# michaelneale/p2p-llm-tunnel

Measured on AMD Instinct MI355X. Metric: tunneled req/s + added p50 TTFT vs direct, mock-LLM SSE at 1/2/4/8 streams, higher is better.
Workload: dtype n/a

## Files before the change

p2p_llm_tunnel_amd/models/server.py:

```python
from __future__ import annotations

import argparse
import asyncio
import functools
import json
import os
import queue
import socket
import sys
import threading
import time
import uuid
from typing import NamedTuple

import torch


class Sampling:
    __slots__ = ("temperature", "top_k", "top_p", "seed")

    def __init__(self, temperature: float = 0.0, top_k: int = 0, top_p: float = 1.0, seed: int | None = None):
        self.temperature = float(temperature)
        self.top_k = int(top_k)
        self.top_p = float(top_p)
# ... 214 lines not shown
        self.h_lp_ids = torch.zeros((rows, MAX_TOP_LOGPROBS), dtype=torch.int32, pin_memory=cuda)
        self.d_lp = self.d_lp_ids = None
        if device is not None:
            self.d_lp = torch.zeros(self.h_lp.shape, dtype=torch.float32, device=device)
            self.d_lp_ids = torch.zeros(self.h_lp_ids.shape, dtype=torch.int32, device=device)
        self.ev = torch.cuda.Event() if cuda else None
        self.n = 0
        self.emits = []
        self.embeds = []
        self.d_emb = self.h_emb = None


class Engine:

    def __init__(self, device="cuda:0", config="tiny", max_batch=8, seed=0, use_graph=True, rows=64, model=None,
                 small_rows=16, prefix_cache=False, prefix_min=16):
        if model is None:
            from p2p_llm_tunnel_amd.models.tiny_llm import TinyLlama
            model = TinyLlama(config, device=device, max_batch=max_batch, seed=seed, fused=True)
        if prefix_cache and not callable(getattr(model, "kv_copy", None)):
            raise ValueError("prefix_cache needs a model with kv_copy(jobs) (slot-to-slot K/V row copy)")
        use_graph = use_graph and model.device.type == "cuda" and hasattr(model, "step_rows")
        max_batch = getattr(model, "max_batch", max_batch)
        if not (1 <= max_batch <= rows and 1 <= small_rows <= rows):
            raise ValueError("need 1 <= max_batch <= rows and small_rows <= rows")
        self.model = model
        self.device = self.model.device
        self.rows = rows
        self.small_rows = small_rows
        self.use_graph = use_graph
        cuda = self.device.type == "cuda"
        self._k = 0
        self._d_last = torch.zeros(max_batch + 1, dtype=torch.int64, device=self.device)
        sizes = [small_rows] + ([rows] if rows > small_rows else []) if use_graph else [rows]
        lp_dev = self.device if use_graph else None
        self._bufs = {R: [_StepBuf(R, cuda, lp_dev), _StepBuf(R, cuda, lp_dev)] for R in sizes}
        self._d_in = {R: torch.zeros((_IN_ROWS, R), dtype=torch.int64, device=self.device) for R in sizes}
        self._graphs = {(R, par, post): self._capture(self._bufs[R][par], 0 if R == small_rows else max_batch, post)
                        for R in sizes if use_graph for par in (0, 1) for post in (0, 1, 2)}
        self.max_batch = max_batch
        self.pending: queue.Queue = queue.Queue()
        self.slots: list[dict | None] = [None] * max_batch
        self.deliver = None
        self._wake = threading.Event()
        self._stop = threading.Event()
# ... 144 lines not shown
            s = self.slots[i]
            s["gen"] += 1
            fin = s["gen"] >= s["req"].max_new or s["pos"] >= max_seq - 1
            emits.append((r, s["req"], fin, s["gen"] - 1))
            if fin:
                done.append(i)
        for pool in pools:
            s = self.slots[pool[0]]
            if s["pos"] >= len(s["ids"]):
                pool[4] = s["req"]
                done.append(pool[0])
        for i in done:
            self.slots[i] = None
        return rows, emits

    def _step_body(self, b: _StepBuf, n: int, run, sample_rows: int = 0, logprobs: bool = False):
        din = self._d_in[b.rows]
        din.copy_(b.h_in, non_blocking=True)
        d = din[:, :n]
        tok = torch.where(d[_DEC] != 0, self._d_last[d[_SLOT]], d[_TOK])
        ids, logits = run(tok, d[_POS].to(torch.int32), d[_SLOT].to(torch.int32))
        if sample_rows:
            from p2p_llm_tunnel_amd import ops
            ops.sample_(logits[:sample_rows], ids[:sample_rows], din[_SMP])
            if logprobs:
                ops.logprobs_(logits[:sample_rows], ids[:sample_rows], din[_LP], b.d_lp[:sample_rows],
                              b.d_lp_ids[:sample_rows])
                b.h_lp.copy_(b.d_lp, non_blocking=True)
                b.h_lp_ids.copy_(b.d_lp_ids, non_blocking=True)
        self._d_last.index_copy_(0, d[_REC], ids)
        b.h_out[:n].copy_(ids, non_blocking=True)

    def _capture(self, b: _StepBuf, emit_rows: int, post: int):
        from p2p_llm_tunnel_amd.models.tiny_llm import capture
        b.np[:] = 0
        b.np[_SLOT, :] = b.np[_REC, :] = self.model.scratch_slot
        run = functools.partial(self.model.step_rows, emit_rows=emit_rows)
        sample_rows = (emit_rows or b.rows) if post else 0
        graph, _ = capture(lambda: self._step_body(b, b.rows, run, sample_rows, post == 2), self.device)
        torch.cuda.synchronize(self.device)
        return graph

    def _launch(self, rows, emits) -> _StepBuf:
        n, scratch = len(rows), self.model.scratch_slot
        R = self.small_rows if self.use_graph and n <= self.small_rows else self.rows
        par = self._k % 2
        self._k += 1
        b = self._bufs[R][par]
        h = b.np
        h[_TOK, :n] = [r.token for r in rows]
        h[_POS, :n] = [r.pos for r in rows]
        h[_SLOT, :n] = [r.slot for r in rows]
        h[_DEC, :n] = [r.decode for r in rows]
        h[_REC, :n] = [r.slot if r.emit else scratch for r in rows]
# ... 672 lines not shown
```

p2p_llm_tunnel_amd/models/tiny_llm.py:

```python
from __future__ import annotations

import math
from dataclasses import dataclass

import torch
import torch.nn.functional as F

from p2p_llm_tunnel_amd import ops


@dataclass(frozen=True)
class LlamaConfig:
    vocab: int = 32000
    dim: int = 1024
    n_layers: int = 4
    n_heads: int = 16
    n_kv_heads: int = 4
    head_dim: int = 64
    ffn: int = 2816
    max_seq: int = 2048
    eps: float = 1e-5
    rope_theta: float = 10000.0
    qk_norm: bool = False
    qkv_bias: bool = False
# ... 131 lines not shown
            if c.qk_norm:
                ws += [L["q_norm"].contiguous(), L["k_norm"].contiguous()]
            if c.qkv_bias:
                ws += [L["bqkv"][head_perm].contiguous()]
        return ws

    def fused_decoder(self) -> ops.FusedLlamaDecoder:
        if self._fused is None:
            c = self.cfg
            dims = ops.LlamaDims(vocab=c.vocab, dim=c.dim, n_layers=c.n_layers, H=c.n_heads, Hkv=c.n_kv_heads,
                                 D=c.head_dim, ffn=c.ffn, max_seq=c.max_seq, max_batch=self.max_batch + 1, eps=c.eps,
                                 theta=c.rope_theta, qk_norm=int(c.qk_norm), qkv_bias=int(c.qkv_bias))
            self._fused = ops.FusedLlamaDecoder(dims, self.fused_weights(), self.k_cache, self.v_cache)
        return self._fused

    def step_rows(self, tokens, pos, slots=None, emit_rows=0, pos_range=None):
        B = tokens.shape[0]
        if self.fused and B <= ops.MAX_ROWS:
            tokens, pos = tokens.contiguous(), pos.contiguous()
            slots = slots.contiguous() if slots is not None else None
            logits = torch.empty(B, self.cfg.vocab, dtype=torch.bfloat16, device=self.device)
            ids = torch.empty(B, dtype=torch.int64, device=self.device)
            self.fused_decoder().step(tokens, pos, logits, ids, slots, emit_rows)
            return ids, logits
        return self._decode_unfused(tokens, pos, pos_range or (0, self.cfg.max_seq - 1))

    def _decode_unfused(self, tokens, pos, pos_range):
        c = self.cfg
        B = tokens.shape[0]
        lens = pos + 1
        x = self.embed.index_select(0, tokens)
# ... 120 lines not shown
```

p2p_llm_tunnel_amd/ops/__init__.py:

```python
from __future__ import annotations

import ctypes
import math
import os

import torch

HERE = os.path.dirname(os.path.abspath(__file__))
_LIB = None


class LlamaDims(ctypes.Structure):
    _fields_ = [(n, ctypes.c_int) for n in ("vocab", "dim", "n_layers", "H", "Hkv", "D", "ffn", "max_seq",
                                           "max_batch")] + [("eps", ctypes.c_float), ("theta", ctypes.c_float),
                                                            ("qk_norm", ctypes.c_int), ("qkv_bias", ctypes.c_int)]


_INT = ctypes.c_int


class GemmPlan(ctypes.Structure):
    _fields_ = [(n, _INT) for n in ("epi", "nw", "tn", "um", "kpl", "grid_x", "grid_y", "ss_in", "M", "N", "K")]


class AttnPlan(ctypes.Structure):
    _fields_ = [(n, _INT) for n in ("D", "G", "slots", "stride", "grid_y")]


class StepPlan(ctypes.Structure):
    _fields_ = ([("rows", _INT), ("emit_rows", _INT)] +
                [(n, GemmPlan) for n in ("qkv_first", "qkv", "o", "gate_up", "down", "lm_head")] +
                [("attn", AttnPlan), ("am_parts", _INT), ("qk_norm_grid", _INT)])


def lib() -> ctypes.CDLL:
    global _LIB
    if _LIB is None:
        path = os.path.join(HERE, os.environ.get("P2PT_HIP_OPS_LIB", "_hip_ops.so"))
        if not os.path.exists(path):
            from . import build as _b
            _b.build()
        _LIB = ctypes.CDLL(path)
        vp, i, f = ctypes.c_void_p, ctypes.c_int, ctypes.c_float
        _LIB.p2pt_rmsnorm.argtypes = [vp, vp, vp, vp, vp, i, i, f, vp]
        _LIB.p2pt_silu_mul.argtypes = [vp, vp, i, i, vp]
        _LIB.p2pt_rope_qkv_cache.argtypes = [vp, vp, vp, vp, vp, i, i, i, i, i, f, vp]
        _LIB.p2pt_qk_norm_rope_cache.argtypes = [vp, vp, vp, vp, vp, vp, vp, vp, i, i, i, i, i, i, f, f, vp]
        _LIB.p2pt_decode_attention.argtypes = [vp, vp, vp, vp, vp, vp, i, i, i, i, i, i, i, f, vp]
        _LIB.p2pt_argmax.argtypes = [vp, vp, i, i, vp]
        _LIB.p2pt_skinny_gemm.argtypes = [vp, vp, vp, i, i, i, vp]
        _LIB.p2pt_sample.argtypes = [vp, vp, vp, i, i, i, vp]
        _LIB.p2pt_logprobs.argtypes = [vp, vp, vp, vp, vp, i, i, vp]
        _LIB.p2pt_kv_copy.argtypes = [vp, vp, i, i, i, i, i, ctypes.POINTER(ctypes.c_int), vp]
        _LIB.p2pt_max_kv_copy_jobs.argtypes = []
        _LIB.p2pt_embed_pool.argtypes = [vp, i, i, vp, vp, i, vp, i, f, i, ctypes.POINTER(ctypes.c_int), vp]
        _LIB.p2pt_max_embed_jobs.argtypes = []
        _LIB.p2pt_llama_ws_bytes.argtypes = [ctypes.POINTER(LlamaDims)]
        _LIB.p2pt_llama_ws_bytes.restype = ctypes.c_size_t
        szp = ctypes.POINTER(ctypes.c_size_t)
        _LIB.p2pt_llama_ws_layout.argtypes = [ctypes.POINTER(LlamaDims), szp, szp, i]
        _LIB.p2pt_llama_ws_layout.restype = ctypes.c_int
        _LIB.p2pt_llama_decode.argtypes = [ctypes.POINTER(LlamaDims), ctypes.POINTER(vp), vp, vp, vp, vp, vp, i, i,
                                           vp, ctypes.c_size_t, vp, vp, vp]
        _LIB.p2pt_llama_plan.argtypes = [ctypes.POINTER(LlamaDims), i, i, ctypes.POINTER(StepPlan)]
        _LIB.p2pt_attn_span.argtypes = [i, i]
        _LIB.p2pt_max_rows.argtypes = []
        _LIB.p2pt_skinny_bench.argtypes = [vp, vp, vp, i, i, i, i, i, i, vp]
        _LIB.p2pt_attn_bench.argtypes = [vp, vp, vp, vp, i, i, i, i, i, vp, vp, vp, vp, i, vp]
        for fn in ("p2pt_rmsnorm", "p2pt_silu_mul", "p2pt_rope_qkv_cache", "p2pt_decode_attention", "p2pt_argmax",
                   "p2pt_skinny_gemm", "p2pt_llama_decode", "p2pt_sample", "p2pt_logprobs", "p2pt_llama_plan", "p2pt_attn_span",
                   "p2pt_max_rows", "p2pt_skinny_bench", "p2pt_attn_bench", "p2pt_kv_copy", "p2pt_max_kv_copy_jobs",
                   "p2pt_embed_pool", "p2pt_max_embed_jobs", "p2pt_qk_norm_rope_cache"):
            getattr(_LIB, fn).restype = ctypes.c_int
        if _LIB.p2pt_max_rows() != MAX_ROWS:
            raise RuntimeError(f"MAX_ROWS = {MAX_ROWS}, but {path} was built for {_LIB.p2pt_max_rows()} rows")
        if _LIB.p2pt_max_kv_copy_jobs() != MAX_KV_COPY_JOBS:
            raise RuntimeError(f"MAX_KV_COPY_JOBS = {MAX_KV_COPY_JOBS}, but {path} was built for "
                               f"{_LIB.p2pt_max_kv_copy_jobs()} jobs")
        if _LIB.p2pt_max_embed_jobs() != MAX_EMBED_JOBS:
            raise RuntimeError(f"MAX_EMBED_JOBS = {MAX_EMBED_JOBS}, but {path} was built for "
                               f"{_LIB.p2pt_max_embed_jobs()} jobs")
    return _LIB


MAX_ROWS = 64
MAX_KV_COPY_JOBS = 8
MAX_EMBED_JOBS = 16
MAX_TOP_LOGPROBS = 20


def step_plan(dims: LlamaDims, B: int, emit_rows: int = 0) -> StepPlan:
    plan = StepPlan()
    if lib().p2pt_llama_plan(ctypes.byref(dims), B, emit_rows, ctypes.byref(plan)) != 0:
        raise ValueError("dims or row count not supported by the fused decode kernels")
    return plan


def attn_span(length: int, slots: int) -> int:
    return lib().p2pt_attn_span(length, slots)


def loaded_path() -> str:
    return lib()._name


def _stream(t: torch.Tensor):
    return ctypes.c_void_p(torch.cuda.current_stream(t.device).cuda_stream)

# ... 164 lines not shown
    _ok(lib().p2pt_decode_attention(_p(q), _p(k_cache), _p(v_cache), _p(lens), _p(out), _p(ws), B, H, Hkv, D, Smax,
                                    nsplit, chunk, scale, _stream(q)), "decode_attention")
    return out


def argmax(logits: torch.Tensor) -> torch.Tensor:
    _check(logits, torch.bfloat16, "logits")
    if logits.dim() != 2:
        raise ValueError("logits must be [B, V]")
    B, V = logits.shape
    out = torch.empty(B, dtype=torch.int64, device=logits.device)
    _ok(lib().p2pt_argmax(_p(logits), _p(out), B, V, _stream(logits)), "argmax")
    return out


def sample_(logits: torch.Tensor, ids: torch.Tensor, params: torch.Tensor) -> torch.Tensor:
    _check(logits, torch.bfloat16, "logits")
    _check(ids, torch.int64, "ids", logits.device)
    _check(params, torch.int64, "params", logits.device)
    if logits.dim() != 2 or ids.shape != (logits.shape[0],) or params.dim() != 2 or params.shape[0] != 5:
        raise ValueError("need logits [B, V], ids [B], params [5, >= B]")
    B, V = logits.shape
    if params.shape[1] < B:
        raise ValueError("params need a column per row")
    _ok(lib().p2pt_sample(_p(logits), _p(ids), _p(params), B, params.shape[1], V, _stream(logits)), "sample")
    return ids


def logprobs_(logits: torch.Tensor, ids: torch.Tensor, want: torch.Tensor, out_lp: torch.Tensor,
              out_ids: torch.Tensor) -> None:
    _check(logits, torch.bfloat16, "logits")
    _check(ids, torch.int64, "ids", logits.device)
    _check(want, torch.int64, "want", logits.device)
    _check(out_lp, torch.float32, "out_lp", logits.device)
    _check(out_ids, torch.int32, "out_ids", logits.device)
    if logits.dim() != 2 or ids.shape != (logits.shape[0],) or want.dim() != 1:
        raise ValueError("need logits [B, V], ids [B], want [>= B]")
    B, V = logits.shape
    if B < 1 or V < 32:
        raise ValueError("need B >= 1 and V >= 32")
# ... 146 lines not shown
                        raise ValueError(f"layer {L}: q_norm and k_norm must be ({dims.D},)")
        elif dims.qkv_bias:
            n_qkv = (dims.H + 2 * dims.Hkv) * dims.D
            for L in range(dims.n_layers):
                if weights[3 + 7 * L + 6].shape != (n_qkv,):
                    raise ValueError(f"layer {L}: bqkv must be ({n_qkv},)")
        nbytes = lib().p2pt_llama_ws_bytes(ctypes.byref(dims))
        if nbytes == 0:
            raise ValueError("model dims not supported by the fused decode kernels")
        self.weights = weights
        self._wptr = (ctypes.c_void_p * len(weights))(*[t.data_ptr() for t in weights])
        self.ws = torch.zeros(nbytes, dtype=torch.uint8, device=dev)
        self.k_cache, self.v_cache = k_cache, v_cache
        self.device = dev
        self._resid = None

    _WS_BUFFERS = (("resid", torch.bfloat16), ("q", torch.bfloat16), ("attn", torch.bfloat16), ("h", torch.bfloat16),
                   ("ss", torch.float32), ("part_o", torch.float32), ("part_ml", torch.float32),
                   ("am_val", torch.float32), ("am_idx", torch.int32), ("counters", torch.int32),
                   ("qkv", torch.bfloat16))

    def workspace_views(self) -> dict:
        d = self.dims
        n = len(self._WS_BUFFERS)
        off, cnt = (ctypes.c_size_t * n)(), (ctypes.c_size_t * n)()
        if lib().p2pt_llama_ws_layout(ctypes.byref(d), off, cnt, n) != n:
            raise RuntimeError("workspace layout: buffer list out of step with decode_fused.hip")
        views = {}
        for (name, dtype), o, c in zip(self._WS_BUFFERS, off, cnt):
            size = torch.empty(0, dtype=dtype).element_size()
# ... 21 lines not shown
        B = tokens.shape[0]
        if slots is not None:
            _check(slots, torch.int32, "slots", self.device)
            if slots.shape != (B,):
                raise ValueError("slots must be [B]")
        limit = MAX_ROWS if slots is not None else min(MAX_ROWS, d.max_batch)
        if not 0 <= emit_rows <= B:
            raise ValueError("emit_rows must be in 0..B")
        if not 1 <= B <= limit or pos.shape != (B,) or ids.shape != (B,):
            raise ValueError(f"rows must be 1..{limit} with matching pos/ids")
        if logits.shape != (B, d.vocab):
            raise ValueError("logits must be [B, vocab]")
        _ok(lib().p2pt_llama_decode(ctypes.byref(d), self._wptr, _p(self.k_cache), _p(self.v_cache), _p(tokens),
                                    _p(pos), _p(slots), B, emit_rows, _p(self.ws), self.ws.numel(), _p(logits),
                                    _p(ids), _stream(tokens)), "llama_decode")
```

p2p_llm_tunnel_amd/ops/decode_fused.hip:

```cpp
#include "decode_fused_kernels.h"

namespace {

struct LlamaDims {
  int vocab, dim, n_layers, H, Hkv, D, ffn, max_seq, max_batch;
  float eps, theta;
  int qk_norm;
  int qkv_bias;
};

constexpr int kTnResid = 1, kTnStore = 2;
constexpr int kCUs = 256;
constexpr int kMaxKpl = 2;

struct GemmPlan {
  int epi, nw, tn, um, kpl;
  int grid_x, grid_y;
  int ss_in;
  int M, N, K;
};
struct AttnPlan {
  int D, G;
  int slots;
  int stride;
  int grid_y;
};
struct StepPlan {
  int rows, emit_rows;
  GemmPlan qkv_first, qkv, o, gate_up, down, lm_head;
  AttnPlan attn;
  int am_parts;
  int qk_norm_grid;
};

GemmPlan plan_gemm(int epi, int tn, int M, int N, int K, bool k_parts = false, int fixed_nw = 0) {
  GemmPlan p{};
  p.epi = epi, p.tn = tn, p.M = M, p.N = N, p.K = K;
  if (k_parts && tn == 1 && (N >> 4) < kCUs) {
    const int kpl = std::min((N >> 3) >= kCUs ? 1 : 2, kMaxKpl);
    if ((M << kpl) <= 16 && K % (32 << kpl) == 0) p.kpl = kpl;
  }
  const int steps = (K >> p.kpl) >> 5;
  if (steps <= 0) return p;
  p.nw = fixed_nw ? fixed_nw : steps <= 16 ? 4 : 8;
  const int per_wave = (steps + p.nw - 1) / p.nw;
  p.um = per_wave <= 1 ? 1 : per_wave <= 2 ? 2 : 4;
  p.grid_x = N / (tn << tile_cwl(p.kpl));
  p.grid_y = (M + 15) >> 4;
  return p;
}

GemmPlan plan_lm_head(const LlamaDims& d, int rows) {
  return plan_gemm(EPI_ARGMAX, kTnStore, rows, d.vocab, d.dim, false, 4);
}

AttnPlan plan_attn(int B, int H, int Hkv, int D, int max_seq) {
  return {D, Hkv > 0 ? H / Hkv : 0, attn_slots(B, Hkv, max_seq), attn_part_stride(max_seq), B * Hkv};
}

StepPlan plan_step(const LlamaDims& d, int B, int emit_rows) {
  StepPlan p{};
  p.rows = B;
  p.emit_rows = emit_rows <= 0 || emit_rows > B ? B : emit_rows;
  p.qkv = plan_gemm(d.qk_norm ? EPI_STORE : d.qkv_bias ? EPI_ROPE_BIAS : EPI_ROPE, 1, B, (d.H + 2 * d.Hkv) * d.D,
                    d.dim);
  if (d.qk_norm) {
    const int per_wg = qknorm_heads_per_wg(d.D);
    p.qk_norm_grid = (d.H + 2 * d.Hkv + per_wg - 1) / per_wg;
  }
  p.attn = plan_attn(B, d.H, d.Hkv, d.D, d.max_seq);
  p.o = plan_gemm(EPI_RESID, kTnResid, B, d.dim, d.H * d.D, true);
  p.gate_up = plan_gemm(EPI_SILU, 1, B, 2 * d.ffn, d.dim);
  p.down = plan_gemm(EPI_RESID, kTnResid, B, d.dim, d.ffn, true);
  p.lm_head = plan_lm_head(d, p.emit_rows);
  p.qkv_first = p.qkv;
  p.qkv_first.ss_in = 1;
  p.gate_up.ss_in = p.o.grid_x;
// ... 183 lines not shown
  const size_t gemm_bytes[] = {size_t(d.vocab) * dim * 2, size_t(d.H + 2 * d.Hkv) * d.D * dim * 2,
                               2 * ffn * dim * 2, dim * hd * 2, dim * ffn * 2};
  for (size_t b : gemm_bytes)
    if (b >= kOob) return false;
  if (d.Hkv <= 0 || d.H % d.Hkv) return false;
  const int gqa = d.H / d.Hkv;
  if (gqa != 1 && gqa != 2 && (gqa < 4 || gqa > 8)) return false;
  if (d.dim % 32 || (d.H * d.D) % 32 || d.ffn % 32) return false;
  if (d.dim % (16 * kTnResid) || d.vocab % (16 * kTnStore) || d.ffn % 16) return false;
  if (d.max_batch <= 0 || d.max_seq <= 0 || d.n_layers <= 0) return false;
  return true;
}

bool rows_ok(int B) { return B > 0 && B <= kMaxM; }

}

extern "C" {

size_t p2pt_llama_ws_bytes(const LlamaDims* d) {
  if (!dims_ok(*d)) return 0;
  return carve(*d, nullptr).bytes;
}

int p2pt_llama_ws_layout(const LlamaDims* d, size_t* off, size_t* count, int n) {
  if (!dims_ok(*d) || n < WS_NBUF) return 0;
  const WsLayout l = ws_layout(*d);
  for (int b = 0; b < WS_NBUF; b++) {
    off[b] = l.off[b];
    count[b] = l.count[b];
  }
  return WS_NBUF;
}

int p2pt_llama_plan(const LlamaDims* d, int B, int emit_rows, StepPlan* out) {
  if (!dims_ok(*d) || !rows_ok(B)) return int(hipErrorInvalidValue);
  *out = plan_step(*d, B, emit_rows);
  return 0;
}

int p2pt_attn_span(int len, int slots) { return len > 0 && slots > 0 ? attn_span(len, unsigned(slots)) : 0; }

int p2pt_max_rows() { return kMaxM; }

int p2pt_llama_decode(const LlamaDims* dp, const void* const* w, void* k_cache, void* v_cache, const int64_t* tokens,
                      const int* pos, const int* slots, int B, int emit_rows, void* ws, size_t ws_bytes, void* logits,
                      int64_t* ids, void* stream) {
  const LlamaDims d = *dp;
  if (!dims_ok(d) || !rows_ok(B) || (!slots && B > d.max_batch)) return int(hipErrorInvalidValue);
  const Workspace W = carve(d, static_cast<uint8_t*>(ws));
  if (ws_bytes < W.bytes) return int(hipErrorInvalidValue);
  const StepPlan P = plan_step(d, B, emit_rows);
  auto s = static_cast<hipStream_t>(stream);
  const size_t layer_cache = size_t(d.max_batch) * d.max_seq * d.Hkv * d.D;
  hipError_t e;
  auto failed = [&](hipError_t r) { return (e = r) != hipSuccess; };

  hipLaunchKernelGGL(k_embed, dim3(B), dim3(256), 0, s, static_cast<const uint16_t*>(w[0]), tokens, W.resid, W.ss,
                     d.dim, d.vocab);
  if (failed(hipGetLastError())) return int(e);
  for (int L = 0; L < d.n_layers; L++) {
    const void* const* wl = w + 3 + (d.qk_norm ? 8 : d.qkv_bias ? 7 : 6) * L;
    uint16_t* kc = static_cast<uint16_t*>(k_cache) + L * layer_cache;
    uint16_t* vc = static_cast<uint16_t*>(v_cache) + L * layer_cache;
    const GemmPlan& qkv = L ? P.qkv : P.qkv_first;
    const GemmArgs to_qkv = d.qk_norm
                                ? gemm(W.resid, wl[1]) + norm(W.ss, qkv.ss_in, d.eps) + store(W.qkv)
                            : d.qkv_bias
                                ? gemm(W.resid, wl[1]) + norm(W.ss, qkv.ss_in, d.eps) +
                                      rope_bias(d, pos, slots, W.q, kc, vc, wl[6])
                                : gemm(W.resid, wl[1]) + norm(W.ss, qkv.ss_in, d.eps) + rope(d, pos, slots, W.q, kc, vc);
    const GemmArgs to_o = gemm(W.attn, wl[2]) + resid(W.resid, W.ss);
    const GemmArgs to_gate_up = gemm(W.resid, wl[4]) + norm(W.ss, P.gate_up.ss_in, d.eps) + store(W.h);
    const GemmArgs to_down = gemm(W.h, wl[5]) + resid(W.resid, W.ss);
    if (failed(launch(qkv, to_qkv, s))) return int(e);
    if (P.qk_norm_grid) {
      const QkNormArgs qn{W.qkv, static_cast<const uint16_t*>(wl[6]), static_cast<const uint16_t*>(wl[7]), pos, slots,
                          d.max_batch, W.q, kc, vc, d.H, d.Hkv, d.max_seq, d.eps, log2f(d.theta)};
      if (failed(launch_qknorm(P.qk_norm_grid, B, d.D, qn, s))) return int(e);
    }
    if (failed(launch_attn(P.attn, W.q, kc, vc, pos, slots, d.max_batch, W.part_o, W.part_ml, W.counters, W.attn, d.H,
                           d.Hkv, d.max_seq, s)))
      return int(e);
    if (failed(launch(P.o, to_o, s))) return int(e);
    if (failed(launch(P.gate_up, to_gate_up, s))) return int(e);
    if (failed(launch(P.down, to_down, s))) return int(e);
  }
  const GemmArgs to_logits =
      gemm(W.resid, w[2]) + norm(W.ss, P.lm_head.ss_in, d.eps) + argmax(logits, W.am_val, W.am_idx);
  if (failed(launch(P.lm_head, to_logits, s))) return int(e);
  hipLaunchKernelGGL(k_argmax_merge, dim3(P.emit_rows), dim3(256), 0, s, W.am_val, W.am_idx, P.am_parts, ids);
  return int(hipGetLastError());
}

int p2pt_skinny_gemm(const void* x, const void* w, void* out, int M, int N, int K, void* stream) {
  if (!rows_ok(M) || N % 32 || K <= 0 || K % 32) return int(hipErrorInvalidValue);
  const GemmPlan p = plan_gemm(EPI_STORE, 2, M, N, K);
  return int(launch(p, gemm(x, w) + store(out), static_cast<hipStream_t>(stream)));
}

int p2pt_qk_norm_rope_cache(const void* qkv, const int* pos, const int* slots, const void* q_weight,
                            const void* k_weight, void* q, void* k_cache, void* v_cache, int B, int H, int Hkv, int D,
                            int Smax, int nslots, float eps, float theta, void* stream) {
  if (!rows_ok(B) || (D != 64 && D != 128) || H <= 0 || Hkv <= 0 || Smax <= 0 || nslots <= 0)
    return int(hipErrorInvalidValue);
  if ((!slots && B > nslots) || !(theta > 0.f)) return int(hipErrorInvalidValue);
  const QkNormArgs a{static_cast<const uint16_t*>(qkv), static_cast<const uint16_t*>(q_weight),
// ... 33 lines not shown
```

p2p_llm_tunnel_amd/ops/decode_fused_kernels.h:

```cpp
#pragma once
#include "bf16_common.h"

#include <algorithm>

namespace {

using namespace p2pt_gpu;

constexpr int kMaxM = 64;

typedef short frag8 __attribute__((ext_vector_type(8)));
typedef float frag4 __attribute__((ext_vector_type(4)));

enum Epi : int { EPI_STORE = 0, EPI_ROPE = 1, EPI_SILU = 2, EPI_RESID = 3, EPI_ARGMAX = 4, EPI_ROPE_BIAS = 5 };

struct GemmArgs {
  const uint16_t* x;
  const uint16_t* w;
  int M, N, K;
  const float* ss_part;
  int ss_parts;
  float eps;
  uint16_t* out;
  float* ss_out;
// ... 286 lines not shown
        if (m >= a.M || !col_ok) continue;
        const float nv = bf_round(rprev[t][r] + bf_round(v[t][r]));
        a.out[size_t(m) * a.N + n] = uint16_t(f2bf_bits(nv));
        sq[r] += nv * nv;
      }
    }
#pragma unroll
    for (int r = 0; r < 4; r++) {
      sq[r] = row16_sum(sq[r]);
      if (c == 0) a.ss_out[bx * kMaxM + mrow0 + r] = sq[r];
    }
  }
}

__global__ __launch_bounds__(256) void k_argmax_merge(const float* __restrict__ am_val, const int* __restrict__ am_idx,
                                                      int parts, int64_t* __restrict__ ids) {
  const int m = blockIdx.x;
  float b = -INFINITY;
  int i = 0x7fffffff;
  for (int p0 = threadIdx.x; p0 < parts; p0 += 8 * 256) {
    float pv[8];
    int pi[8];
#pragma unroll
    for (int j = 0; j < 8; j++) {
      const int p = p0 + j * 256;
      pv[j] = p < parts ? am_val[p * kMaxM + m] : -INFINITY;
      pi[j] = p < parts ? am_idx[p * kMaxM + m] : 0x7fffffff;
    }
#pragma unroll
    for (int j = 0; j < 8; j++)
      if (pv[j] > b || (pv[j] == b && pi[j] < i)) {
// ... 3 lines not shown
  }
  wave_argmax(b, i);
  __shared__ float sb[4];
  __shared__ int si[4];
  if ((threadIdx.x & 63) == 0) {
    sb[threadIdx.x >> 6] = b;
    si[threadIdx.x >> 6] = i;
  }
  __syncthreads();
  if (threadIdx.x == 0) {
    for (int w = 1; w < 4; w++)
      if (sb[w] > b || (sb[w] == b && si[w] < i)) {
        b = sb[w];
        i = si[w];
      }
    ids[m] = i == 0x7fffffff ? 0 : i;
  }
}

__global__ __launch_bounds__(256) void k_embed(const uint16_t* __restrict__ embed, const int64_t* __restrict__ tok,
                                               uint16_t* __restrict__ resid, float* __restrict__ ss_out, int dim,
                                               int vocab) {
  const int b = blockIdx.x;
  int64_t t = tok[b];
  t = t < 0 ? 0 : (t >= vocab ? vocab - 1 : t);
  const uint4* src = reinterpret_cast<const uint4*>(embed + size_t(t) * dim);
  uint4* dst = reinterpret_cast<uint4*>(resid + size_t(b) * dim);
  float ss = 0.f;
  for (int i = threadIdx.x; i < dim / 8; i += 256) {
    const uint4 v = src[i];
    dst[i] = v;
    float f[8];
    unpack8(v, f);
#pragma unroll
    for (int j = 0; j < 8; j++) ss += f[j] * f[j];
  }
  __shared__ float red[4];
  ss = wave_sum(ss);
  if ((threadIdx.x & 63) == 0) red[threadIdx.x >> 6] = ss;
  __syncthreads();
  if (threadIdx.x == 0) ss_out[b] = red[0] + red[1] + red[2] + red[3];
}

struct QkNormArgs {
  const uint16_t* qkv;
  const uint16_t* gq;
  const uint16_t* gk;
  const int* pos;
  const int* slot;
  int nslots;
  uint16_t* q_out;
  uint16_t* kc;
  uint16_t* vc;
  int H, Hkv, Smax;
  float eps, log2_theta;
};
// ... 278 lines not shown
```

p2p_llm_tunnel_amd/ops/sample.hip:

```cpp
#include "bf16_common.h"

namespace {

using namespace p2pt_gpu;

constexpr int kThreads = 1024, kWaves = kThreads / 64;

__device__ __forceinline__ uint32_t okey(float f) {
  uint32_t u = __float_as_uint(f);
  return (u & 0x80000000u) ? ~u : (u | 0x80000000u);
}

__device__ __forceinline__ uint64_t mix64(uint64_t z) {
  z = (z ^ (z >> 30)) * 0xBF58476D1CE4E5B9ull;
  z = (z ^ (z >> 27)) * 0x94D049BB133111EBull;
  return z ^ (z >> 31);
}

__device__ __forceinline__ float gumbel(uint64_t seed, uint64_t ctr, uint32_t i) {
  uint64_t h = mix64(seed + mix64(ctr * 0x9E3779B97F4A7C15ull + i + 1));
  double u = (double(h >> 11) + 0.5) * (1.0 / 9007199254740992.0);
  return float(-log(-log(u)));
}

// ... 45 lines not shown
#pragma unroll
    for (int q = 0; q < 4; q++) {
      if (run + v[q] >= need || q == 3) {
        dg = 255 - 4 * lane - q;
        ab = run;
        break;
      }
      run += v[q];
    }
    *digit_out = dg;
    *above_out = ab;
  }
}

__global__ __launch_bounds__(kThreads) void k_sample(const uint16_t* __restrict__ logits, int64_t* __restrict__ ids,
                                                     const int64_t* __restrict__ params, int ld, int V) {
  const int row = blockIdx.x;
  const int B = ld;
  const float T = __uint_as_float(uint32_t(params[row]));
  if (!(T >= 1e-4f)) return;
  int64_t k = params[B + row];
  float p = __uint_as_float(uint32_t(params[2 * B + row]));
  const uint64_t seed = uint64_t(params[3 * B + row]), ctr = uint64_t(params[4 * B + row]);
  if (k <= 0 || k > V) k = V;
  if (!(p > 0.f && p < 1.f)) p = 1.f;
  const float invT = 1.0f / T;
  const uint16_t* lr = logits + size_t(row) * V;

  __shared__ float red[kWaves];
  __shared__ uint32_t hist_u[256];
  __shared__ float hist_f[256];
  __shared__ int s_digit;
  __shared__ uint32_t s_above_u;
  __shared__ float s_above_f;
  __shared__ float s_best[kWaves];
// ... 57 lines not shown
  int bi = 0x7fffffff;
  for (int i = threadIdx.x; i < V; i += kThreads) {
    const float zi = bf2f(lr[i]) * invT;
    if (okey(zi) < cut) continue;
    am_take(best, bi, zi + gumbel(seed, ctr, uint32_t(i)), i);
  }
  wave_argmax(best, bi);
  if ((threadIdx.x & 63) == 0) {
    s_best[threadIdx.x >> 6] = best;
    s_bi[threadIdx.x >> 6] = bi;
  }
  __syncthreads();
  if (threadIdx.x == 0) {
    for (int w = 1; w < kWaves; w++) am_take(best, bi, s_best[w], s_bi[w]);
    if (bi != 0x7fffffff) ids[row] = bi;
  }
}

}

extern "C" {

int p2pt_sample(const void* logits, int64_t* ids, const int64_t* params, int B, int ld, int V, void* stream) {
  if (B <= 0 || V <= 0 || ld < B) return int(hipErrorInvalidValue);
  hipLaunchKernelGGL(k_sample, dim3(B), dim3(kThreads), 0, static_cast<hipStream_t>(stream),
                     static_cast<const uint16_t*>(logits), ids, params, ld, V);
  return int(hipGetLastError());
}

}
```

Baseline: 15.97.

## Fold token gather, int32 casts and last-token record into fused decode kernels

Adds a staged decode path in which the embed kernel reads the raw int64 staging block directly. It picks the decode token from the last-token buffer and writes int32 pos/slot rows itself. The argmax-merge or sample kernel then scatters the chosen id back into the last-token buffer. This removes the separate torch.where/gather, dtype cast and index_copy kernels from each captured graph step, so fewer launches run per step. It is on by default when graphs are used, and it adds a new code path with duplicated record logic in the argmax and sample kernels.

Measured after the change: 15.97. No clear change (-0.0%).

```diff
diff --git a/p2p_llm_tunnel_amd/models/server.py b/p2p_llm_tunnel_amd/models/server.py
--- a/p2p_llm_tunnel_amd/models/server.py
+++ b/p2p_llm_tunnel_amd/models/server.py
@@ -252,7 +252,7 @@
 class Engine:
 
     def __init__(self, device="cuda:0", config="tiny", max_batch=8, seed=0, use_graph=True, rows=64, model=None,
-                 small_rows=16, prefix_cache=False, prefix_min=16):
+                 small_rows=16, prefix_cache=False, prefix_min=16, native_step=True):
         if model is None:
             from p2p_llm_tunnel_amd.models.tiny_llm import TinyLlama
             model = TinyLlama(config, device=device, max_batch=max_batch, seed=seed, fused=True)
@@ -267,6 +267,7 @@
         self.rows = rows
         self.small_rows = small_rows
         self.use_graph = use_graph
+        self.native_step = bool(native_step) and use_graph
         cuda = self.device.type == "cuda"
         self._k = 0
         self._d_last = torch.zeros(max_batch + 1, dtype=torch.int64, device=self.device)
@@ -441,21 +442,29 @@
             self.slots[i] = None
         return rows, emits
 
-    def _step_body(self, b: _StepBuf, n: int, run, sample_rows: int = 0, logprobs: bool = False):
+    def _step_body(self, b: _StepBuf, n: int, run, sample_rows: int = 0, logprobs: bool = False,
+                   native: bool = False):
         din = self._d_in[b.rows]
         din.copy_(b.h_in, non_blocking=True)
         d = din[:, :n]
-        tok = torch.where(d[_DEC] != 0, self._d_last[d[_SLOT]], d[_TOK])
-        ids, logits = run(tok, d[_POS].to(torch.int32), d[_SLOT].to(torch.int32))
+        if native:
+            ids, logits = run(None, None, staged=(din, self._d_last, not sample_rows))
+        else:
+            tok = torch.where(d[_DEC] != 0, self._d_last[d[_SLOT]], d[_TOK])
+            ids, logits = run(tok, d[_POS].to(torch.int32), d[_SLOT].to(torch.int32))
         if sample_rows:
             from p2p_llm_tunnel_amd import ops
-            ops.sample_(logits[:sample_rows], ids[:sample_rows], din[_SMP])
+            if native:
+                ops.sample_(logits[:sample_rows], ids[:sample_rows], din[_SMP], din[_REC], self._d_last)
+            else:
+                ops.sample_(logits[:sample_rows], ids[:sample_rows], din[_SMP])
             if logprobs:
                 ops.logprobs_(logits[:sample_rows], ids[:sample_rows], din[_LP], b.d_lp[:sample_rows],
                               b.d_lp_ids[:sample_rows])
                 b.h_lp.copy_(b.d_lp, non_blocking=True)
                 b.h_lp_ids.copy_(b.d_lp_ids, non_blocking=True)
-        self._d_last.index_copy_(0, d[_REC], ids)
+        if not native:
+            self._d_last.index_copy_(0, d[_REC], ids)
         b.h_out[:n].copy_(ids, non_blocking=True)
 
     def _capture(self, b: _StepBuf, emit_rows: int, post: int):
@@ -464,7 +473,8 @@
         b.np[_SLOT, :] = b.np[_REC, :] = self.model.scratch_slot
         run = functools.partial(self.model.step_rows, emit_rows=emit_rows)
         sample_rows = (emit_rows or b.rows) if post else 0
-        graph, _ = capture(lambda: self._step_body(b, b.rows, run, sample_rows, post == 2), self.device)
+        graph, _ = capture(lambda: self._step_body(b, b.rows, run, sample_rows, post == 2, self.native_step),
+                           self.device)
         torch.cuda.synchronize(self.device)
         return graph
 
diff --git a/p2p_llm_tunnel_amd/models/tiny_llm.py b/p2p_llm_tunnel_amd/models/tiny_llm.py
--- a/p2p_llm_tunnel_amd/models/tiny_llm.py
+++ b/p2p_llm_tunnel_amd/models/tiny_llm.py
@@ -169,7 +169,16 @@
             self._fused = ops.FusedLlamaDecoder(dims, self.fused_weights(), self.k_cache, self.v_cache)
         return self._fused
 
-    def step_rows(self, tokens, pos, slots=None, emit_rows=0, pos_range=None):
+    def step_rows(self, tokens, pos, slots=None, emit_rows=0, pos_range=None, staged=None):
+        if staged is not None:
+            block, last, record = staged
+            B = block.shape[1]
+            if not (self.fused and B <= ops.MAX_ROWS):
+                raise ValueError(f"a staged step needs the fused path and at most {ops.MAX_ROWS} rows")
+            logits = torch.empty(B, self.cfg.vocab, dtype=torch.bfloat16, device=self.device)
+            ids = torch.empty(B, dtype=torch.int64, device=self.device)
+            self.fused_decoder().step_staged(block, last, logits, ids, emit_rows, record)
+            return ids, logits
         B = tokens.shape[0]
         if self.fused and B <= ops.MAX_ROWS:
             tokens, pos = tokens.contiguous(), pos.contiguous()
diff --git a/p2p_llm_tunnel_amd/ops/__init__.py b/p2p_llm_tunnel_amd/ops/__init__.py
--- a/p2p_llm_tunnel_amd/ops/__init__.py
+++ b/p2p_llm_tunnel_amd/ops/__init__.py
@@ -30,7 +30,7 @@
 class StepPlan(ctypes.Structure):
     _fields_ = ([("rows", _INT), ("emit_rows", _INT)] +
                 [(n, GemmPlan) for n in ("qkv_first", "qkv", "o", "gate_up", "down", "lm_head")] +
-                [("attn", AttnPlan), ("am_parts", _INT), ("qk_norm_grid", _INT)])
+                [("attn", AttnPlan), ("am_parts", _INT), ("qk_norm_grid", _INT), ("staged", _INT)])
 
 
 def lib() -> ctypes.CDLL:
@@ -50,6 +50,7 @@
         _LIB.p2pt_argmax.argtypes = [vp, vp, i, i, vp]
         _LIB.p2pt_skinny_gemm.argtypes = [vp, vp, vp, i, i, i, vp]
         _LIB.p2pt_sample.argtypes = [vp, vp, vp, i, i, i, vp]
+        _LIB.p2pt_sample_record.argtypes = [vp, vp, vp, vp, vp, i, i, i, vp]
         _LIB.p2pt_logprobs.argtypes = [vp, vp, vp, vp, vp, i, i, vp]
         _LIB.p2pt_kv_copy.argtypes = [vp, vp, i, i, i, i, i, ctypes.POINTER(ctypes.c_int), vp]
         _LIB.p2pt_max_kv_copy_jobs.argtypes = []
@@ -62,7 +63,10 @@
         _LIB.p2pt_llama_ws_layout.restype = ctypes.c_int
         _LIB.p2pt_llama_decode.argtypes = [ctypes.POINTER(LlamaDims), ctypes.POINTER(vp), vp, vp, vp, vp, vp, i, i,
                                            vp, ctypes.c_size_t, vp, vp, vp]
+        _LIB.p2pt_llama_decode_staged.argtypes = [ctypes.POINTER(LlamaDims), ctypes.POINTER(vp), vp, vp, vp, i, vp, vp,
+                                                  i, i, i, vp, ctypes.c_size_t, vp, vp, vp]
         _LIB.p2pt_llama_plan.argtypes = [ctypes.POINTER(LlamaDims), i, i, ctypes.POINTER(StepPlan)]
+        _LIB.p2pt_llama_plan_staged.argtypes = [ctypes.POINTER(LlamaDims), i, i, ctypes.POINTER(StepPlan)]
         _LIB.p2pt_attn_span.argtypes = [i, i]
         _LIB.p2pt_max_rows.argtypes = []
         _LIB.p2pt_skinny_bench.argtypes = [vp, vp, vp, i, i, i, i, i, i, vp]
@@ -70,7 +74,8 @@
         for fn in ("p2pt_rmsnorm", "p2pt_silu_mul", "p2pt_rope_qkv_cache", "p2pt_decode_attention", "p2pt_argmax",
                    "p2pt_skinny_gemm", "p2pt_llama_decode", "p2pt_sample", "p2pt_logprobs", "p2pt_llama_plan", "p2pt_attn_span",
                    "p2pt_max_rows", "p2pt_skinny_bench", "p2pt_attn_bench", "p2pt_kv_copy", "p2pt_max_kv_copy_jobs",
-                   "p2pt_embed_pool", "p2pt_max_embed_jobs", "p2pt_qk_norm_rope_cache"):
+                   "p2pt_embed_pool", "p2pt_max_embed_jobs", "p2pt_qk_norm_rope_cache", "p2pt_llama_decode_staged",
+                   "p2pt_llama_plan_staged", "p2pt_sample_record"):
             getattr(_LIB, fn).restype = ctypes.c_int
         if _LIB.p2pt_max_rows() != MAX_ROWS:
             raise RuntimeError(f"MAX_ROWS = {MAX_ROWS}, but {path} was built for {_LIB.p2pt_max_rows()} rows")
@@ -89,9 +94,10 @@
 MAX_TOP_LOGPROBS = 20
 
 
-def step_plan(dims: LlamaDims, B: int, emit_rows: int = 0) -> StepPlan:
+def step_plan(dims: LlamaDims, B: int, emit_rows: int = 0, staged: bool = False) -> StepPlan:
     plan = StepPlan()
-    if lib().p2pt_llama_plan(ctypes.byref(dims), B, emit_rows, ctypes.byref(plan)) != 0:
+    fn = lib().p2pt_llama_plan_staged if staged else lib().p2pt_llama_plan
+    if fn(ctypes.byref(dims), B, emit_rows, ctypes.byref(plan)) != 0:
         raise ValueError("dims or row count not supported by the fused decode kernels")
     return plan
 
@@ -286,7 +292,8 @@
     return out
 
 
-def sample_(logits: torch.Tensor, ids: torch.Tensor, params: torch.Tensor) -> torch.Tensor:
+def sample_(logits: torch.Tensor, ids: torch.Tensor, params: torch.Tensor, rec: torch.Tensor | None = None,
+            last: torch.Tensor | None = None) -> torch.Tensor:
     _check(logits, torch.bfloat16, "logits")
     _check(ids, torch.int64, "ids", logits.device)
     _check(params, torch.int64, "params", logits.device)
@@ -295,7 +302,15 @@
     B, V = logits.shape
     if params.shape[1] < B:
         raise ValueError("params need a column per row")
-    _ok(lib().p2pt_sample(_p(logits), _p(ids), _p(params), B, params.shape[1], V, _stream(logits)), "sample")
+    if (rec is None) != (last is None):
+        raise ValueError("rec and last go together")
+    if rec is not None:
+        _check(rec, torch.int64, "rec", logits.device)
+        _check(last, torch.int64, "last", logits.device)
+        if rec.dim() != 1 or rec.shape[0] < B or last.dim() != 1 or last.shape[0] < 1:
+            raise ValueError("need rec [>= B] and last [slots >= 1]")
+    _ok(lib().p2pt_sample_record(_p(logits), _p(ids), _p(params), _p(rec), _p(last), B, params.shape[1], V,
+                                 _stream(logits)), "sample")
     return ids
 
 
@@ -472,6 +487,7 @@
         self.k_cache, self.v_cache = k_cache, v_cache
         self.device = dev
         self._resid = None
+        self.rows32 = torch.zeros((3, MAX_ROWS), dtype=torch.int32, device=dev)
 
     _WS_BUFFERS = (("resid", torch.bfloat16), ("q", torch.bfloat16), ("attn", torch.bfloat16), ("h", torch.bfloat16),
                    ("ss", torch.float32), ("part_o", torch.float32), ("part_ml", torch.float32),
@@ -523,3 +539,24 @@
         _ok(lib().p2pt_llama_decode(ctypes.byref(d), self._wptr, _p(self.k_cache), _p(self.v_cache), _p(tokens),
                                     _p(pos), _p(slots), B, emit_rows, _p(self.ws), self.ws.numel(), _p(logits),
                                     _p(ids), _stream(tokens)), "llama_decode")
+
+    def step_staged(self, staged: torch.Tensor, last: torch.Tensor, logits: torch.Tensor, ids: torch.Tensor,
+                    emit_rows: int = 0, record: bool = True) -> None:
+        d = self.dims
+        _check(staged, torch.int64, "staged", self.device)
+        _check(last, torch.int64, "last", self.device)
+        _check(logits, torch.bfloat16, "logits", self.device)
+        _check(ids, torch.int64, "ids", self.device)
+        if staged.dim() != 2 or staged.shape[0] < 5 or not 1 <= staged.shape[1] <= MAX_ROWS:
+            raise ValueError(f"staged must be [>= 5, 1..{MAX_ROWS}]")
+        B = staged.shape[1]
+        if last.shape != (d.max_batch,):
+            raise ValueError(f"last must be [{d.max_batch}] (one entry per cache slot)")
+        if not 0 <= emit_rows <= B:
+            raise ValueError("emit_rows must be in 0..B")
+        if ids.shape != (B,) or logits.shape != (B, d.vocab):
+            raise ValueError("need ids [B] and logits [B, vocab]")
+        _ok(lib().p2pt_llama_decode_staged(ctypes.byref(d), self._wptr, _p(self.k_cache), _p(self.v_cache),
+                                           _p(staged), B, _p(last), _p(self.rows32), int(bool(record)), B, emit_rows, _p(self.ws),
+                                           self.ws.numel(), _p(logits), _p(ids), _stream(staged)),
+            "llama_decode_staged")
diff --git a/p2p_llm_tunnel_amd/ops/decode_fused.hip b/p2p_llm_tunnel_amd/ops/decode_fused.hip
--- a/p2p_llm_tunnel_amd/ops/decode_fused.hip
+++ b/p2p_llm_tunnel_amd/ops/decode_fused.hip
@@ -31,6 +31,7 @@
   AttnPlan attn;
   int am_parts;
   int qk_norm_grid;
+  int staged;
 };
 
 GemmPlan plan_gemm(int epi, int tn, int M, int N, int K, bool k_parts = false, int fixed_nw = 0) {
@@ -58,9 +59,10 @@
   return {D, Hkv > 0 ? H / Hkv : 0, attn_slots(B, Hkv, max_seq), attn_part_stride(max_seq), B * Hkv};
 }
 
-StepPlan plan_step(const LlamaDims& d, int B, int emit_rows) {
+StepPlan plan_step(const LlamaDims& d, int B, int emit_rows, bool staged = false) {
   StepPlan p{};
   p.rows = B;
+  p.staged = staged;
   p.emit_rows = emit_rows <= 0 || emit_rows > B ? B : emit_rows;
   p.qkv = plan_gemm(d.qk_norm ? EPI_STORE : d.qkv_bias ? EPI_ROPE_BIAS : EPI_ROPE, 1, B, (d.H + 2 * d.Hkv) * d.D,
                     d.dim);
@@ -274,51 +276,33 @@
 
 bool rows_ok(int B) { return B > 0 && B <= kMaxM; }
 
-}
-
-extern "C" {
-
-size_t p2pt_llama_ws_bytes(const LlamaDims* d) {
-  if (!dims_ok(*d)) return 0;
-  return carve(*d, nullptr).bytes;
-}
-
-int p2pt_llama_ws_layout(const LlamaDims* d, size_t* off, size_t* count, int n) {
-  if (!dims_ok(*d) || n < WS_NBUF) return 0;
-  const WsLayout l = ws_layout(*d);
-  for (int b = 0; b < WS_NBUF; b++) {
-    off[b] = l.off[b];
-    count[b] = l.count[b];
-  }
-  return WS_NBUF;
-}
-
-int p2pt_llama_plan(const LlamaDims* d, int B, int emit_rows, StepPlan* out) {
-  if (!dims_ok(*d) || !rows_ok(B)) return int(hipErrorInvalidValue);
-  *out = plan_step(*d, B, emit_rows);
-  return 0;
-}
-
-int p2pt_attn_span(int len, int slots) { return len > 0 && slots > 0 ? attn_span(len, unsigned(slots)) : 0; }
-
-int p2pt_max_rows() { return kMaxM; }
-
-int p2pt_llama_decode(const LlamaDims* dp, const void* const* w, void* k_cache, void* v_cache, const int64_t* tokens,
-                      const int* pos, const int* slots, int B, int emit_rows, void* ws, size_t ws_bytes, void* logits,
-                      int64_t* ids, void* stream) {
-  const LlamaDims d = *dp;
-  if (!dims_ok(d) || !rows_ok(B) || (!slots && B > d.max_batch)) return int(hipErrorInvalidValue);
-  const Workspace W = carve(d, static_cast<uint8_t*>(ws));
-  if (ws_bytes < W.bytes) return int(hipErrorInvalidValue);
-  const StepPlan P = plan_step(d, B, emit_rows);
-  auto s = static_cast<hipStream_t>(stream);
+struct StepRows {
+  const int64_t* tokens;
+  const int* pos;
+  const int* slots;
+  const int64_t* staged;
+  int ld;
+  int64_t* last;
+  int* rows32;
+  bool record;
+};
+
+hipError_t run_step(const LlamaDims& d, const StepPlan& P, const Workspace& W, const void* const* w, void* k_cache,
+                    void* v_cache, const StepRows& rows, void* logits, int64_t* ids, hipStream_t s) {
+  const int B = P.rows;
   const size_t layer_cache = size_t(d.max_batch) * d.max_seq * d.Hkv * d.D;
+  const int* pos = P.staged ? rows.rows32 + RB_POS * kMaxM : rows.pos;
+  const int* slots = P.staged ? rows.rows32 + RB_SLOT * kMaxM : rows.slots;
   hipError_t e;
   auto failed = [&](hipError_t r) { return (e = r) != hipSuccess; };
 
-  hipLaunchKernelGGL(k_embed, dim3(B), dim3(256), 0, s, static_cast<const uint16_t*>(w[0]), tokens, W.resid, W.ss,
-                     d.dim, d.vocab);
-  if (failed(hipGetLastError())) return int(e);
+  if (P.staged)
+    hipLaunchKernelGGL(k_embed_staged, dim3(B), dim3(256), 0, s, static_cast<const uint16_t*>(w[0]), rows.staged,
+                       rows.ld, rows.last, rows.rows32, W.resid, W.ss, d.dim, d.vocab);
+  else
+    hipLaunchKernelGGL(k_embed, dim3(B), dim3(256), 0, s, static_cast<const uint16_t*>(w[0]), rows.tokens, W.resid,
+                       W.ss, d.dim, d.vocab);
+  if (failed(hipGetLastError())) return e;
   for (int L = 0; L < d.n_layers; L++) {
     const void* const* wl = w + 3 + (d.qk_norm ? 8 : d.qkv_bias ? 7 : 6) * L;
     uint16_t* kc = static_cast<uint16_t*>(k_cache) + L * layer_cache;
@@ -333,24 +317,87 @@
     const GemmArgs to_o = gemm(W.attn, wl[2]) + resid(W.resid, W.ss);
     const GemmArgs to_gate_up = gemm(W.resid, wl[4]) + norm(W.ss, P.gate_up.ss_in, d.eps) + store(W.h);
     const GemmArgs to_down = gemm(W.h, wl[5]) + resid(W.resid, W.ss);
-    if (failed(launch(qkv, to_qkv, s))) return int(e);
+    if (failed(launch(qkv, to_qkv, s))) return e;
     if (P.qk_norm_grid) {
       const QkNormArgs qn{W.qkv, static_cast<const uint16_t*>(wl[6]), static_cast<const uint16_t*>(wl[7]), pos, slots,
                           d.max_batch, W.q, kc, vc, d.H, d.Hkv, d.max_seq, d.eps, log2f(d.theta)};
-      if (failed(launch_qknorm(P.qk_norm_grid, B, d.D, qn, s))) return int(e);
+      if (failed(launch_qknorm(P.qk_norm_grid, B, d.D, qn, s))) return e;
     }
     if (failed(launch_attn(P.attn, W.q, kc, vc, pos, slots, d.max_batch, W.part_o, W.part_ml, W.counters, W.attn, d.H,
                            d.Hkv, d.max_seq, s)))
-      return int(e);
-    if (failed(launch(P.o, to_o, s))) return int(e);
-    if (failed(launch(P.gate_up, to_gate_up, s))) return int(e);
-    if (failed(launch(P.down, to_down, s))) return int(e);
+      return e;
+    if (failed(launch(P.o, to_o, s))) return e;
+    if (failed(launch(P.gate_up, to_gate_up, s))) return e;
+    if (failed(launch(P.down, to_down, s))) return e;
   }
   const GemmArgs to_logits =
       gemm(W.resid, w[2]) + norm(W.ss, P.lm_head.ss_in, d.eps) + argmax(logits, W.am_val, W.am_idx);
-  if (failed(launch(P.lm_head, to_logits, s))) return int(e);
-  hipLaunchKernelGGL(k_argmax_merge, dim3(P.emit_rows), dim3(256), 0, s, W.am_val, W.am_idx, P.am_parts, ids);
-  return int(hipGetLastError());
+  if (failed(launch(P.lm_head, to_logits, s))) return e;
+  const bool record = P.staged && rows.record;
+  hipLaunchKernelGGL(k_argmax_merge, dim3(P.emit_rows), dim3(256), 0, s, W.am_val, W.am_idx, P.am_parts, ids,
+                     record ? rows.staged + ST_REC * rows.ld : nullptr, record ? rows.last : nullptr);
+  return hipGetLastError();
+}
+
+}
+
+extern "C" {
+
+size_t p2pt_llama_ws_bytes(const LlamaDims* d) {
+  if (!dims_ok(*d)) return 0;
+  return carve(*d, nullptr).bytes;
+}
+
+int p2pt_llama_ws_layout(const LlamaDims* d, size_t* off, size_t* count, int n) {
+  if (!dims_ok(*d) || n < WS_NBUF) return 0;
+  const WsLayout l = ws_layout(*d);
+  for (int b = 0; b < WS_NBUF; b++) {
+    off[b] = l.off[b];
+    count[b] = l.count[b];
+  }
+  return WS_NBUF;
+}
+
+int p2pt_llama_plan(const LlamaDims* d, int B, int emit_rows, StepPlan* out) {
+  if (!dims_ok(*d) || !rows_ok(B)) return int(hipErrorInvalidValue);
+  *out = plan_step(*d, B, emit_rows);
+  return 0;
+}
+
+int p2pt_attn_span(int len, int slots) { return len > 0 && slots > 0 ? attn_span(len, unsigned(slots)) : 0; }
+
+int p2pt_max_rows() { return kMaxM; }
+
+int p2pt_llama_decode(const LlamaDims* dp, const void* const* w, void* k_cache, void* v_cache, const int64_t* tokens,
+                      const int* pos, const int* slots, int B, int emit_rows, void* ws, size_t ws_bytes, void* logits,
+                      int64_t* ids, void* stream) {
+  const LlamaDims d = *dp;
+  if (!dims_ok(d) || !rows_ok(B) || (!slots && B > d.max_batch)) return int(hipErrorInvalidValue);
+  const Workspace W = carve(d, static_cast<uint8_t*>(ws));
+  if (ws_bytes < W.bytes) return int(hipErrorInvalidValue);
+  StepRows rows{};
+  rows.tokens = tokens, rows.pos = pos, rows.slots = slots;
+  return int(run_step(d, plan_step(d, B, emit_rows), W, w, k_cache, v_cache, rows, logits, ids,
+                      static_cast<hipStream_t>(stream)));
+}
+
+int p2pt_llama_plan_staged(const LlamaDims* d, int B, int emit_rows, StepPlan* out) {
+  if (!dims_ok(*d) || !rows_ok(B)) return int(hipErrorInvalidValue);
+  *out = plan_step(*d, B, emit_rows, true);
+  return 0;
+}
+
+int p2pt_llama_decode_staged(const LlamaDims* dp, const void* const* w, void* k_cache, void* v_cache,
+                             const int64_t* staged, int ld, int64_t* last, int* rows32, int record, int B,
+                             int emit_rows, void* ws, size_t ws_bytes, void* logits, int64_t* ids, void* stream) {
+  const LlamaDims d = *dp;
+  if (!dims_ok(d) || !rows_ok(B) || ld < B || !staged || !last || !rows32) return int(hipErrorInvalidValue);
+  const Workspace W = carve(d, static_cast<uint8_t*>(ws));
+  if (ws_bytes < W.bytes) return int(hipErrorInvalidValue);
+  StepRows rows{};
+  rows.staged = staged, rows.ld = ld, rows.last = last, rows.rows32 = rows32, rows.record = record != 0;
+  return int(run_step(d, plan_step(d, B, emit_rows, true), W, w, k_cache, v_cache, rows, logits, ids,
+                      static_cast<hipStream_t>(stream)));
 }
 
 int p2pt_skinny_gemm(const void* x, const void* w, void* out, int M, int N, int K, void* stream) {
diff --git a/p2p_llm_tunnel_amd/ops/decode_fused_kernels.h b/p2p_llm_tunnel_amd/ops/decode_fused_kernels.h
--- a/p2p_llm_tunnel_amd/ops/decode_fused_kernels.h
+++ b/p2p_llm_tunnel_amd/ops/decode_fused_kernels.h
@@ -324,7 +324,8 @@
 }
 
 __global__ __launch_bounds__(256) void k_argmax_merge(const float* __restrict__ am_val, const int* __restrict__ am_idx,
-                                                      int parts, int64_t* __restrict__ ids) {
+                                                      int parts, int64_t* __restrict__ ids,
+                                                      const int64_t* __restrict__ rec, int64_t* __restrict__ last) {
   const int m = blockIdx.x;
   float b = -INFINITY;
   int i = 0x7fffffff;
@@ -358,15 +359,15 @@
         b = sb[w];
         i = si[w];
       }
-    ids[m] = i == 0x7fffffff ? 0 : i;
-  }
-}
-
-__global__ __launch_bounds__(256) void k_embed(const uint16_t* __restrict__ embed, const int64_t* __restrict__ tok,
-                                               uint16_t* __restrict__ resid, float* __restrict__ ss_out, int dim,
-                                               int vocab) {
-  const int b = blockIdx.x;
-  int64_t t = tok[b];
+    const int64_t id = i == 0x7fffffff ? 0 : i;
+    ids[m] = id;
+    if (last) last[rec[m]] = id;
+  }
+}
+
+__device__ __forceinline__ void embed_row(const uint16_t* __restrict__ embed, int64_t t, int b,
+                                          uint16_t* __restrict__ resid, float* __restrict__ ss_out, int dim,
+                                          int vocab) {
   t = t < 0 ? 0 : (t >= vocab ? vocab - 1 : t);
   const uint4* src = reinterpret_cast<const uint4*>(embed + size_t(t) * dim);
   uint4* dst = reinterpret_cast<uint4*>(resid + size_t(b) * dim);
@@ -384,6 +385,31 @@
   if ((threadIdx.x & 63) == 0) red[threadIdx.x >> 6] = ss;
   __syncthreads();
   if (threadIdx.x == 0) ss_out[b] = red[0] + red[1] + red[2] + red[3];
+}
+
+__global__ __launch_bounds__(256) void k_embed(const uint16_t* __restrict__ embed, const int64_t* __restrict__ tok,
+                                               uint16_t* __restrict__ resid, float* __restrict__ ss_out, int dim,
+                                               int vocab) {
+  embed_row(embed, tok[blockIdx.x], blockIdx.x, resid, ss_out, dim, vocab);
+}
+
+enum StagedRow : int { ST_TOK = 0, ST_POS = 1, ST_SLOT = 2, ST_DEC = 3, ST_REC = 4, ST_NROWS = 5 };
+enum RowsBuf : int { RB_TOK = 0, RB_POS = 1, RB_SLOT = 2, RB_NROWS = 3 };
+
+__global__ __launch_bounds__(256) void k_embed_staged(const uint16_t* __restrict__ embed,
+                                                      const int64_t* __restrict__ staged, int ld,
+                                                      const int64_t* __restrict__ last, int* __restrict__ rows32,
+                                                      uint16_t* __restrict__ resid, float* __restrict__ ss_out,
+                                                      int dim, int vocab) {
+  const int b = blockIdx.x;
+  const int64_t slot = staged[ST_SLOT * ld + b], dec = staged[ST_DEC * ld + b], own = staged[ST_TOK * ld + b];
+  const int64_t t = dec != 0 ? last[slot] : own;
+  if (threadIdx.x == 0) {
+    rows32[RB_TOK * kMaxM + b] = int(t);
+    rows32[RB_POS * kMaxM + b] = int(staged[ST_POS * ld + b]);
+    rows32[RB_SLOT * kMaxM + b] = int(slot);
+  }
+  embed_row(embed, t, b, resid, ss_out, dim, vocab);
 }
 
 struct QkNormArgs {
diff --git a/p2p_llm_tunnel_amd/ops/sample.hip b/p2p_llm_tunnel_amd/ops/sample.hip
--- a/p2p_llm_tunnel_amd/ops/sample.hip
+++ b/p2p_llm_tunnel_amd/ops/sample.hip
@@ -83,11 +83,15 @@
 }
 
 __global__ __launch_bounds__(kThreads) void k_sample(const uint16_t* __restrict__ logits, int64_t* __restrict__ ids,
-                                                     const int64_t* __restrict__ params, int ld, int V) {
+                                                     const int64_t* __restrict__ params, int ld, int V,
+                                                     const int64_t* __restrict__ rec, int64_t* __restrict__ last) {
   const int row = blockIdx.x;
   const int B = ld;
   const float T = __uint_as_float(uint32_t(params[row]));
-  if (!(T >= 1e-4f)) return;
+  if (!(T >= 1e-4f)) {
+    if (last && threadIdx.x == 0) last[rec[row]] = ids[row];
+    return;
+  }
   int64_t k = params[B + row];
   float p = __uint_as_float(uint32_t(params[2 * B + row]));
   const uint64_t seed = uint64_t(params[3 * B + row]), ctr = uint64_t(params[4 * B + row]);
@@ -175,6 +179,7 @@
   if (threadIdx.x == 0) {
     for (int w = 1; w < kWaves; w++) am_take(best, bi, s_best[w], s_bi[w]);
     if (bi != 0x7fffffff) ids[row] = bi;
+    if (last) last[rec[row]] = bi != 0x7fffffff ? int64_t(bi) : ids[row];
   }
 }
 
@@ -182,11 +187,16 @@
 
 extern "C" {
 
+int p2pt_sample_record(const void* logits, int64_t* ids, const int64_t* params, const int64_t* rec, int64_t* last,
+                       int B, int ld, int V, void* stream) {
+  if (B <= 0 || V <= 0 || ld < B || (rec == nullptr) != (last == nullptr)) return int(hipErrorInvalidValue);
+  hipLaunchKernelGGL(k_sample, dim3(B), dim3(kThreads), 0, static_cast<hipStream_t>(stream),
+                     static_cast<const uint16_t*>(logits), ids, params, ld, V, rec, last);
+  return int(hipGetLastError());
+}
+
 int p2pt_sample(const void* logits, int64_t* ids, const int64_t* params, int B, int ld, int V, void* stream) {
-  if (B <= 0 || V <= 0 || ld < B) return int(hipErrorInvalidValue);
-  hipLaunchKernelGGL(k_sample, dim3(B), dim3(kThreads), 0, static_cast<hipStream_t>(stream),
-                     static_cast<const uint16_t*>(logits), ids, params, ld, V);
-  return int(hipGetLastError());
-}
-
-}
+  return p2pt_sample_record(logits, ids, params, nullptr, nullptr, B, ld, V, stream);
+}
+
+}
```
